# DanEngelbrecht/longtail

Hardware: AMD Instinct MI355X
Metric: ingest GB/s (chunk+hash+compress) (higher is better)
Workload: dtype u8/u32

## Files before the change

longtail_amd/csrc/k_lz4.hip:

```cpp
#include "k_copy.h"
#include "lthip_internal.h"

#include <string>

#include <stdlib.h>

namespace
{

struct Lz4Block
{
    uint64_t src_off;
    uint64_t dst_off;
    uint32_t size;
    uint32_t dst_cap;
    uint32_t seg_base;
    uint32_t nseg;
    uint32_t grp_base;
    uint32_t ngrp;
    uint32_t cgrp_base;
    uint32_t ncgrp;
};

struct Lz4Meta
// ... 115 lines not shown
        uint4 o;
        if constexpr (PAD)
        {
            const uint32_t w = b >> 2, sh = b & 3u;
            uint32_t d[4];
            lds_run<true, 4>(sdata, w, d);
            const uint32_t d4 = lds_dw<true>(sdata, w + 4u);
            o.x = __builtin_amdgcn_alignbyte(d[1], d[0], sh);
            o.y = __builtin_amdgcn_alignbyte(d[2], d[1], sh);
            o.z = __builtin_amdgcn_alignbyte(d[3], d[2], sh);
            o.w = __builtin_amdgcn_alignbyte(d4, d[3], sh);
        }
        else
        {
            o.x = lds_read32(sdata, b);
            o.y = lds_read32(sdata, b + 4u);
            o.z = lds_read32(sdata, b + 8u);
            o.w = lds_read32(sdata, b + 12u);
        }
        *reinterpret_cast<uint4*>(dst + (uint64_t)v * 16u) = o;
    }
    const uint32_t done = nvec << 4;
    if ((uint32_t)lane < n - done)
        dst[done + (uint32_t)lane] = (uint8_t)lds_byte<PAD>(sdata, sbyte + done + (uint32_t)lane);
}

__device__ __forceinline__ void emit_len(uint8_t* out, uint32_t len, int lane)
{
    const uint32_t n = len / 255u + 1u;
    for (uint32_t j = lane; j < n; j += 64)
        out[j] = j + 1 == n ? (uint8_t)(len % 255u) : (uint8_t)255;
}

struct Lz4Seq
{
    uint32_t op;
    uint32_t anchor;
    uint32_t first_lit;
    uint32_t first_hdr;
    uint32_t nseq;
    bool have_first;
};

template <int FMT>
__device__ __forceinline__ void lz4_coop_sequence(const uint8_t* __restrict__ sbytes, uint32_t head, uint8_t* __restrict__ out,
                                                  uint64_t* __restrict__ recs, int lane, uint32_t end_limit, uint32_t pf, uint32_t cf,
                                                  uint32_t mlen, bool extend_fwd, bool extend_back, Lz4Seq& st)
{
    if (extend_fwd || extend_back)
    {
        const uint32_t room = extend_back ? (pf - st.anchor < cf ? pf - st.anchor : cf) : 0u;
        uint32_t nf, nb;
        {
            const uint32_t j = (uint32_t)lane & 31u;
            const bool fwd = lane < 32;
            const uint32_t a1 = fwd ? pf + mlen + j : pf - 1u - j;
            const uint32_t a2 = fwd ? cf + mlen + j : cf - 1u - j;
            const bool inr = fwd ? (extend_fwd && a1 < end_limit) : j < room;
            bool same = false;
            if (inr)
                same = sbytes[a1 + head] == sbytes[a2 + head];
            const uint64_t diff = __builtin_amdgcn_ballot_w64(!same);
            const uint32_t dl = (uint32_t)diff, dh = (uint32_t)(diff >> 32);
            nf = dl ? (uint32_t)__builtin_ctz(dl) : 32u;
            nb = dh ? (uint32_t)__builtin_ctz(dh) : 32u;
        }
        mlen += nf;
        if (nf == 32u)
        {
            const uint32_t* sdata = reinterpret_cast<const uint32_t*>(sbytes);
            for (;;)
            {
                const uint32_t i = pf + mlen + 4u * (uint32_t)lane;
                uint32_t cnt = 0;
                if (i < end_limit)
                {
                    const uint32_t x = lds_read32(sdata, i + head) ^ lds_read32(sdata, cf + mlen + 4u * (uint32_t)lane + head);
                    const uint32_t lim = end_limit - i < 4u ? end_limit - i : 4u;
                    cnt = x ? (uint32_t)__builtin_ctz(x) >> 3 : 4u;
                    cnt = cnt < lim ? cnt : lim;
                }
                const uint64_t diff = __builtin_amdgcn_ballot_w64(cnt < 4u);
                if (diff)
                {
                    const int f = __builtin_ctzll(diff);
                    mlen += 4u * (uint32_t)f + __builtin_amdgcn_readlane(cnt, f);
                    break;
                }
                mlen += 256u;
            }
        }
        if (nb == 32u && room > 32u)
        {
            uint32_t back = 32u;
            for (;;)
            {
                const uint32_t j = back + (uint32_t)lane;
                const bool same = j < room && sbytes[pf - 1u - j + head] == sbytes[cf - 1u - j + head];
                const uint64_t diff = __builtin_amdgcn_ballot_w64(!same);
                if (diff)
                {
                    back += (uint32_t)__builtin_ctzll(diff);
                    break;
                }
                back += 64u;
            }
            nb = back;
        }
        pf -= nb;
        cf -= nb;
        mlen += nb;
    }
    const uint32_t lit = pf - st.anchor;
    const uint32_t mcode = mlen - 4u;
    const uint32_t off = pf - cf;
    if constexpr (FMT == 1)
    {
        for (uint32_t j = lane; j < lit; j += 64)
            out[st.op + j] = sbytes[st.anchor + j + head];
        if (lane == 0)
            recs[st.nseq] = (uint64_t)lit | ((uint64_t)mlen << 16) | ((uint64_t)off << 32);
        st.have_first = true;
        st.nseq += 1u;
        st.op += lit;
        st.anchor = pf + mlen;
        return;
    }
    const uint32_t hdr = 1u + lz4_len_bytes(lit);
    const uint32_t mext = lz4_len_bytes(mcode);
    const uint32_t total = hdr + lit + 2u + mext;
    const uint32_t token = ((lit < 15u ? lit : 15u) << 4) | (mcode < 15u ? mcode : 15u);
    for (uint32_t j = lane; j < total; j += 64)
    {
        uint32_t b;
        if (j >= hdr && j < hdr + lit)
            b = sbytes[st.anchor + (j - hdr) + head];
        else if (j == 0)
            b = token;
        else if (j < hdr)
            b = j + 1 == hdr ? (lit - 15u) % 255u : 255u;
        else if (j == hdr + lit)
            b = off & 255u;
        else if (j == hdr + lit + 1u)
            b = off >> 8;
        else
            b = j + 1 == total ? (mcode - 15u) % 255u : 255u;
        out[st.op + j] = (uint8_t)b;
    }
    if (!st.have_first)
    {
        st.have_first = true;
        st.first_lit = lit;
        st.first_hdr = hdr;
    }
    st.op += total;
    st.anchor = pf + mlen;
}

constexpr int LZ4_G_BATCH = 8;
constexpr int LZ4_G_LANES = 16;
constexpr int LZ4_PROBE_BATCHES = 4;
constexpr uint32_t LZ4_Z_CHAIN = LTHIP_ZSTD_CHAIN;
constexpr uint32_t Z_PIECE = 128u << 10;
constexpr int LZ4_TAB_LZ4 = 1024 + 256;
constexpr int LZ4_TAB_ZSTD = 1024 + 256;
[[maybe_unused]] constexpr int LZ4_TAB_LANES = 2560;
constexpr int LZ4_TAB_SHARED = 1536, LZ4_SH_LOG2 = 13;

#include "lz4/lz4_lane_parse.inc"
#include "lz4/lz4_classify.inc"
#include "lz4/lz4_lanes_kernel.inc"
#include "lz4/lz4_stitch.inc"


}


extern "C" size_t lthip_lz4_bound(size_t size) { return size > 0x7E000000u ? 0 : size + size / 255 + 16; }

static int upload_blocks(lthip_ctx* ctx, uint32_t block_count, const uint64_t* src_offsets, const uint32_t* src_sizes,
                         const uint64_t* dst_offsets, const uint32_t* dst_caps, uint32_t seg_bytes, uint32_t gunits, Lz4Block** d_blocks,
                         uint64_t* out_nseg, uint64_t* out_ngrp = nullptr, uint64_t* out_ncgrp = nullptr)
{
    std::vector<Lz4Block> hb(block_count);
    uint64_t nseg = 0, ngrp = 0, ncgrp = 0;
    for (uint32_t b = 0; b < block_count; ++b)
    {
        if (src_sizes[b] > 0x7E000000u)
            return lthip_fail(ctx, EINVAL, "lz4", "block larger than LZ4_MAX_INPUT_SIZE");
        hb[b].src_off = src_offsets[b];
        hb[b].dst_off = dst_offsets[b];
        hb[b].size = src_sizes[b];
        hb[b].dst_cap = dst_caps[b];
        hb[b].seg_base = (uint32_t)nseg;
        hb[b].nseg = seg_bytes ? (uint32_t)(((uint64_t)src_sizes[b] + seg_bytes - 1) / seg_bytes) : 0;
        hb[b].grp_base = (uint32_t)ngrp;
        hb[b].ngrp = (hb[b].nseg + gunits - 1) / gunits;
        ngrp += hb[b].ngrp;
        hb[b].cgrp_base = (uint32_t)ncgrp;
        hb[b].ncgrp = (hb[b].nseg + LZ4_G_BATCH - 1) / LZ4_G_BATCH;
        ncgrp += hb[b].ncgrp;
        nseg += hb[b].nseg;
    }
    if (nseg > 0x7FFFFFF0ull)
        return lthip_fail(ctx, EINVAL, "lz4", "too many segments in one batch");
    void* p;
    int err = lthip_scratch(ctx, S_LZ4_BLOCKS, sizeof(Lz4Block) * (size_t)block_count, &p);
    if (err)
        return err;
    if ((err = lthip_stage_upload(ctx, p, hb.data(), sizeof(Lz4Block) * (size_t)block_count, ctx->stream)))
        return err;
    *d_blocks = (Lz4Block*)p;
    *out_nseg = nseg;
    if (out_ngrp)
        *out_ngrp = ngrp;
    if (out_ncgrp)
        *out_ncgrp = ncgrp;
    return 0;
}

#ifdef LTHIP_K5_PROF
extern "C" __attribute__((visibility("default"))) int lthip_k5_prof_dump(int reset)
{
    unsigned long long h[32];
    if (hipMemcpyFromSymbol(h, HIP_SYMBOL(g_k5_prof), sizeof(h)) != hipSuccess)
        return -1;
    static const char* names[16] = {"stage+clear+barrier", "prefetch issue", "pre-seed", "loop: probe", "loop: extend fwd/back", "loop: long+record",
                                    "cover scans", "emission", "unit end", "group barrier", "#probe iterations", "#extension rounds", "#hits", "#long matches", "", ""};
    unsigned long long tot = 0;
    for (int i = 0; i < 10; ++i)
        tot += h[i];
    for (int i = 0; i < 14; ++i)
        printf("k5prof %-24s %14llu%s\n", names[i], h[i], i < 10 ? (std::string("  ") + std::to_string(100.0 * (double)h[i] / (double)(tot ? tot : 1)).substr(0, 5) + " %").c_str() : "");
    if (reset)
    {
        memset(h, 0, sizeof(h));
        (void)hipMemcpyToSymbol(HIP_SYMBOL(g_k5_prof), h, sizeof(h));
    }
    return 0;
}
#endif

static bool lz4_lane_parser()
{
#ifdef LTHIP_ABLATIONS
    static const bool v = [] {
        const char* e = getenv("LTHIP_LZ4_PARSER");
        return !(e && strcmp(e, "batch") == 0);
    }();
    return v;
#else
    return true;
#endif
}

template <int FMT, int CLS>
static int launch_segments(lthip_ctx* ctx, uint32_t groups, uint32_t SEG, const void* d_src, const Lz4Block* d_blocks, uint32_t block_count,
                           uint32_t g0, uint8_t* streams, Lz4Meta* meta, uint64_t* zrecs, uint8_t* spec_dst, uint32_t dbg, uint32_t ngroups,
                           uint32_t* worklist)
{
    constexpr int TAB = FMT == 1 ? LZ4_TAB_ZSTD : LZ4_TAB_LZ4;
    const size_t lds = (size_t)lz4_window_lds_bytes(LZ4_G_BATCH * SEG + 64u, false) + 16 + (size_t)LZ4_G_BATCH * TAB * 2;
    if (lds > 64u * 1024u && !ctx->k5_lds_enabled[FMT][CLS])
    {
        LTHIP_CHECK(ctx, hipFuncSetAttribute(reinterpret_cast<const void*>(&k_lz4_segments<LZ4_G_BATCH, TAB, FMT, CLS>),
                                             hipFuncAttributeMaxDynamicSharedMemorySize, 160 * 1024));
        ctx->k5_lds_enabled[FMT][CLS] = true;
    }
    hipLaunchKernelGGL((k_lz4_segments<LZ4_G_BATCH, TAB, FMT, CLS>), dim3(groups), dim3(64 * LZ4_G_BATCH), lds, ctx->stream, (const uint8_t*)d_src,
                       d_blocks, block_count, g0, SEG, streams, meta, zrecs, spec_dst, dbg, nullptr, ngroups, worklist);
    LTHIP_LAUNCH_CHECK(ctx);
    return 0;
}

#ifdef LTHIP_ABLATIONS
template <int TAB, int FMT, int SH = 0, int PV = 0>
static int launch_segments_lane_mode(lthip_ctx* ctx, uint32_t groups, uint32_t SEG, const void* d_src, const Lz4Block* d_blocks, uint32_t block_count,
                                     uint8_t* streams, Lz4Meta* meta, uint64_t* zrecs, uint8_t* spec_dst, uint32_t dbg, uint64_t* lane_recs,
                                     uint32_t ngroups, uint32_t* worklist)
{
    constexpr int G = LZ4_G_LANES;
    const size_t lds = (size_t)lz4_window_lds_bytes(G * SEG + 64u + (PV == 2 ? LZ4_LPAD : 0u), PV == 2) + 16 + (size_t)G * TAB * 2 + (SH ? (size_t)4 << SH : 0);
    static bool granted[64] = {};
    if (ctx->device < 0 || ctx->device >= 64 || !granted[ctx->device])
    {
        LTHIP_CHECK(ctx, hipFuncSetAttribute(reinterpret_cast<const void*>(&k_lz4_segments_modes<G, TAB, FMT, 1, 0, SH, PV>),
                                             hipFuncAttributeMaxDynamicSharedMemorySize, 160 * 1024));
        if (ctx->device >= 0 && ctx->device < 64)
            granted[ctx->device] = true;
    }
    int ncu = 256;
    (void)hipDeviceGetAttribute(&ncu, hipDeviceAttributeMultiprocessorCount, ctx->device);
    const uint32_t grid = groups < (uint32_t)ncu ? groups : (uint32_t)ncu;
    hipLaunchKernelGGL((k_lz4_segments_modes<G, TAB, FMT, 1, 0, SH, PV>), dim3(grid), dim3(64 * G), lds, ctx->stream, (const uint8_t*)d_src, d_blocks,
                       block_count, 0u, SEG, streams, meta, zrecs, spec_dst, dbg, lane_recs, ngroups, worklist);
    LTHIP_LAUNCH_CHECK(ctx);
    return 0;
}
#endif

template <int FMT>
static int launch_match_finder(lthip_ctx* ctx, bool lanes, uint32_t SEG, const void* d_src, const Lz4Block* d_blocks, uint32_t block_count,
                               uint32_t g0, uint32_t g1, uint64_t ngrp, uint64_t ncgrp, uint8_t* streams, Lz4Meta* meta, uint64_t* zrecs,
                               uint8_t* spec_dst, uint32_t dbg, [[maybe_unused]] uint64_t* lane_recs)
{
    if (!lanes)
        return launch_segments<FMT, 0>(ctx, g1 - g0, SEG, d_src, d_blocks, block_count, g0, streams, meta, zrecs, spec_dst, dbg, 0, nullptr);
#ifdef LTHIP_ABLATIONS
    LTHIP_ABLATION_ENV(env_shared, "LTHIP_LZ4_SHARED");
    const bool shared = env_shared.get() != 0;
    LTHIP_ABLATION_ENV(env_pv, "LTHIP_LZ4_PV");
    const bool pv2 = shared && env_pv.get() != 0;
    if (dbg & 16384u)
        return pv2      ? launch_segments_lane_mode<LZ4_TAB_SHARED, FMT, LZ4_SH_LOG2, 2>(ctx, (uint32_t)ngrp, SEG, d_src, d_blocks, block_count, streams, meta, zrecs,
                                                                                        spec_dst, dbg, lane_recs, (uint32_t)ngrp, nullptr)
               : shared ? launch_segments_lane_mode<LZ4_TAB_SHARED, FMT, LZ4_SH_LOG2>(ctx, (uint32_t)ngrp, SEG, d_src, d_blocks, block_count, streams, meta, zrecs,
                                                                                     spec_dst, dbg, lane_recs, (uint32_t)ngrp, nullptr)
                        : launch_segments_lane_mode<LZ4_TAB_LANES, FMT>(ctx, (uint32_t)ngrp, SEG, d_src, d_blocks, block_count, streams, meta, zrecs, spec_dst,
                                                                        dbg, lane_recs, (uint32_t)ngrp, nullptr);
#endif
    void* wl;
    int err = lthip_scratch(ctx, S_LZ4_CLASSIFY, 4 * (11 * (size_t)ngrp + 16), &wl);
    if (err)
        return err;
    LTHIP_CHECK(ctx, hipMemsetAsync(wl, 0, 4 * (2 * (size_t)ngrp + 4), ctx->stream));
    if ((err = launch_segments<FMT, 1>(ctx, (uint32_t)ncgrp, SEG, d_src, d_blocks, block_count, 0, streams, meta, zrecs, spec_dst, dbg, (uint32_t)ngrp,
                                       (uint32_t*)wl)))
        return err;
#ifdef LTHIP_ABLATIONS
    LTHIP_ABLATION_ENV(env_halves, "LTHIP_LZ4_HALVES");
    if (!pv2 || env_halves.get() == 0)
        return pv2      ? launch_segments_lane_mode<LZ4_TAB_SHARED, FMT, LZ4_SH_LOG2, 2>(ctx, (uint32_t)ngrp, SEG, d_src, d_blocks, block_count, streams, meta, zrecs,
                                                                                        spec_dst, dbg, lane_recs, (uint32_t)ngrp, (uint32_t*)wl)
               : shared ? launch_segments_lane_mode<LZ4_TAB_SHARED, FMT, LZ4_SH_LOG2>(ctx, (uint32_t)ngrp, SEG, d_src, d_blocks, block_count, streams, meta, zrecs,
                                                                                     spec_dst, dbg, lane_recs, (uint32_t)ngrp, (uint32_t*)wl)
                        : launch_segments_lane_mode<LZ4_TAB_LANES, FMT>(ctx, (uint32_t)ngrp, SEG, d_src, d_blocks, block_count, streams, meta, zrecs, spec_dst,
                                                                        dbg, lane_recs, (uint32_t)ngrp, (uint32_t*)wl);
#endif
    const uint32_t nthreads = 256, ng = (uint32_t)ngrp;
    uint32_t hist = (FMT == 1 && (dbg & LZ4_DBG_Q_MAX)) ? 3u : (FMT == 1 && (dbg & LZ4_DBG_Q_HIGH)) ? 1u : 0u;
    int ncu = 256;
    (void)hipDeviceGetAttribute(&ncu, hipDeviceAttributeMultiprocessorCount, ctx->device);
    LTHIP_ABLATION_ENV(env_far, "LTHIP_LZ4_FAR");
    const uint32_t farlog = env_far.get() >= 0 ? (uint32_t)env_far.get() : (10u | (12u << 8) | (8u << 16));
#ifdef LTHIP_ABLATIONS
    LTHIP_ABLATION_ENV(env_split, "LTHIP_LZ4_SPLITWG");
    if (env_split.get() > 0 && hist == 0u)
    {
        hist = 2u;
        hipLaunchKernelGGL(k_lz4_pair_halves, dim3((ng + nthreads - 1) / nthreads), dim3(nthreads), 0, ctx->stream, (uint32_t*)wl, ng, 0u, d_blocks, block_count, hist);
        hipLaunchKernelGGL(k_lz4_pair_halves, dim3((2u * ng + nthreads) / nthreads), dim3(nthreads), 0, ctx->stream, (uint32_t*)wl, ng, 1u, d_blocks, block_count, hist);
        LTHIP_LAUNCH_CHECK(ctx);
        const size_t lds8 = (size_t)lz4_window_lds_bytes(8u * SEG + 64u + LZ4_LPAD + 32u, true) + 16 + (size_t)8 * LZ4_TAB_SHARED * 2 + ((size_t)2 << LZ4_SH_LOG2);
        static bool granted8[2] = {false, false};
        if (!granted8[FMT])
        {
            LTHIP_CHECK(ctx, hipFuncSetAttribute(reinterpret_cast<const void*>(&k_lz4_lanes2<FMT, 8>), hipFuncAttributeMaxDynamicSharedMemorySize, 160 * 1024));
            granted8[FMT] = true;
        }
        hipLaunchKernelGGL((k_lz4_lanes2<FMT, 8>), dim3(2u * (uint32_t)ncu), dim3(64 * 8), lds8, ctx->stream, (const uint8_t*)d_src, d_blocks, block_count, SEG,
                           streams, meta, zrecs, spec_dst, dbg, ng, (uint32_t*)wl, farlog);
        LTHIP_LAUNCH_CHECK(ctx);
        return 0;
    }
#endif
    hipLaunchKernelGGL(k_lz4_pair_halves, dim3((ng + nthreads - 1) / nthreads), dim3(nthreads), 0, ctx->stream, (uint32_t*)wl, ng, 0u, d_blocks, block_count, hist);
    hipLaunchKernelGGL(k_lz4_pair_halves, dim3((ng / 2 + nthreads) / nthreads), dim3(nthreads), 0, ctx->stream, (uint32_t*)wl, ng, 1u, d_blocks, block_count, hist);
    LTHIP_LAUNCH_CHECK(ctx);
    const size_t lds = (size_t)lz4_window_lds_bytes(LZ4_G_LANES * SEG + 64u + LZ4_LPAD + 32u, true) + 16 + (size_t)LZ4_G_LANES * LZ4_TAB_SHARED * 2 +
                       ((size_t)4 << LZ4_SH_LOG2);
    if (!ctx->k5h_lds_enabled[FMT])
    {
        LTHIP_CHECK(ctx, hipFuncSetAttribute(reinterpret_cast<const void*>(&k_lz4_lanes2<FMT>), hipFuncAttributeMaxDynamicSharedMemorySize, 160 * 1024));
        ctx->k5h_lds_enabled[FMT] = true;
    }
    hipLaunchKernelGGL((k_lz4_lanes2<FMT>), dim3((uint32_t)ncu), dim3(64 * LZ4_G_LANES), lds, ctx->stream, (const uint8_t*)d_src, d_blocks,
                       block_count, SEG, streams, meta, zrecs, spec_dst, dbg, ng, (uint32_t*)wl, farlog);
    LTHIP_LAUNCH_CHECK(ctx);
    return 0;
}

static int lz4_compress_batch(lthip_ctx* ctx, const void* d_src, uint32_t block_count, const uint64_t* src_offsets,
                              const uint32_t* src_sizes, void* d_dst, const uint64_t* dst_offsets, const uint32_t* dst_caps,
                              uint32_t* d_out_sizes, int segment_log2);

uint64_t lthip_codec_batch_bytes()
{
    static const uint64_t v = [] {
        const char* e = getenv("LTHIP_BATCH_BYTES");
        const uint64_t x = e ? strtoull(e, nullptr, 10) : 0;
        return x ? x : (8ull << 30);
    }();
    return v;
}

uint64_t lthip_origin_budget_mib()
{
    static LthipEnvInt env_org{"LTHIP_ORIGIN_MIB"};
    if (env_org.get() > 0)
        return (uint64_t)env_org.get();
    static const uint64_t v = [] {
        size_t free_b = 0, total_b = 0;
        if (hipMemGetInfo(&free_b, &total_b) != hipSuccess)
            return (uint64_t)4096;
        uint64_t mib = (uint64_t)(free_b >> 20) / 4u;
        mib = mib < 4096u ? 4096u : mib > 16384u ? 16384u : mib;
        return mib;
    }();
    return v;
}

extern "C" int lthip_lz4_compress_blocks(lthip_ctx* ctx, const void* d_src, uint32_t block_count, const uint64_t* src_offsets,
                                         const uint32_t* src_sizes, void* d_dst, const uint64_t* dst_offsets,
                                         const uint32_t* dst_caps, uint32_t* d_out_sizes, int segment_log2)
{
    if (!ctx || !d_out_sizes || (block_count && (!src_offsets || !src_sizes || !dst_offsets || !dst_caps || !d_dst)))
        return EINVAL;
    const uint64_t budget = lthip_codec_batch_bytes();
    for (uint32_t b0 = 0; b0 < block_count;)
    {
        uint64_t bytes = src_sizes[b0];
        uint32_t b1 = b0 + 1;
        while (b1 < block_count && bytes + src_sizes[b1] <= budget)
            bytes += src_sizes[b1++];
        const int err = lz4_compress_batch(ctx, d_src, b1 - b0, src_offsets + b0, src_sizes + b0, d_dst, dst_offsets + b0, dst_caps + b0,
                                           d_out_sizes + b0, segment_log2);
        if (err)
            return err;
        b0 = b1;
    }
    return 0;
}

static int lz4_compress_batch(lthip_ctx* ctx, const void* d_src, uint32_t block_count, const uint64_t* src_offsets,
                              const uint32_t* src_sizes, void* d_dst, const uint64_t* dst_offsets, const uint32_t* dst_caps,
                              uint32_t* d_out_sizes, int segment_log2)
{
    if (segment_log2 == 0)
        segment_log2 = 12;
    if (segment_log2 < 10 || segment_log2 > 13)
        return lthip_fail(ctx, EINVAL, "lz4", "segment_log2 (unit size) must be 0 (default = 12) or 10..13");
    const uint32_t SEG = 1u << segment_log2;
    LTHIP_CHECK(ctx, hipSetDevice(ctx->device));
    Lz4Block* d_blocks = nullptr;
    uint64_t nseg64 = 0, ngrp64 = 0;
    const bool lanes = lz4_lane_parser() && SEG == 4096u;
    const uint32_t GU = lanes ? LZ4_G_LANES : LZ4_G_BATCH;
    uint64_t ncgrp64 = 0;
    int err = upload_blocks(ctx, block_count, src_offsets, src_sizes, dst_offsets, dst_caps, SEG, GU, &d_blocks, &nseg64, &ngrp64, &ncgrp64);
    if (err)
        return err;
    const uint32_t nseg = (uint32_t)nseg64;
    void *meta, *plan, *bout, *streams, *runs, *lrecs = nullptr;
    if (lanes && (err = lthip_scratch(ctx, S_LZ4_LANE_RECS, (size_t)64 * LZ4_LANE_MAXREC * 8 * ((size_t)nseg + 1), &lrecs)))
        return err;
    if ((err = lthip_scratch(ctx, S_TABLES2, 4 * ((size_t)nseg + block_count + 1), &runs)))
        return err;
    if ((err = lthip_scratch(ctx, S_LZ4_META, sizeof(Lz4Meta) * ((size_t)nseg + 1), &meta)))
        return err;
    if ((err = lthip_scratch(ctx, S_LZ4_SEGS, sizeof(Lz4Plan) * ((size_t)nseg + 1), &plan)))
        return err;
    if ((err = lthip_scratch(ctx, S_MISC, sizeof(Lz4BlockOut) * (size_t)block_count, &bout)))
        return err;
    if ((err = lthip_scratch(ctx, S_LZ4_STREAM, (size_t)lz4_stream_stride(SEG) * ((size_t)nseg + 1), &streams)))
        return err;
    LTHIP_ABLATION_ENV(env_dbg, "LTHIP_LZ4_DBG");
    const uint32_t dbg = env_dbg.get() > 0 ? (uint32_t)env_dbg.get() : 0u;
    uint64_t total_bytes = 0;
    for (uint32_t b = 0; b < block_count; ++b)
        total_bytes += src_sizes[b];
    const uint32_t want = (!(dbg & 32u) || lanes) ? 1u : (total_bytes >= (1ull << 30) ? 4u : (total_bytes >= (256ull << 20) ? 2u : 1u));
    std::vector<uint32_t> cut{0};
    {
        uint64_t acc = 0;
        for (uint32_t b = 0; b < block_count; ++b)
        {
            acc += src_sizes[b];
            if (cut.size() < want && acc * want >= total_bytes * cut.size() && b + 1 < block_count)
                cut.push_back(b + 1);
        }
        cut.push_back(block_count);
    }
    std::vector<uint32_t> grp_first(block_count + 1, 0);
    for (uint32_t b = 0; b < block_count; ++b)
        grp_first[b + 1] = grp_first[b] + (uint32_t)(((((uint64_t)src_sizes[b] + SEG - 1) / SEG) + GU - 1) / GU);
    const bool overlap = cut.size() > 2;
    void* worklist;
    if ((err = lthip_scratch(ctx, S_LZ4_WORKLIST, 4 * (2 * (size_t)ngrp64 + 1) * (cut.size() - 1), &worklist)))
        return err;
    int ncu = 256;
    (void)hipDeviceGetAttribute(&ncu, hipDeviceAttributeMultiprocessorCount, ctx->device);
    LTHIP_ABLATION_ENV(env_swg, "LTHIP_LZ4_STITCH_WGS");
    int stitch_wgs = 7;
    if (hipOccupancyMaxActiveBlocksPerMultiprocessor(&stitch_wgs, k_lz4_stitch_copy, K6_THREADS, 0) != hipSuccess || stitch_wgs < 1)
        stitch_wgs = 7;
    const uint32_t copy_grid = (uint32_t)ncu * (env_swg.get() > 0 ? (uint32_t)env_swg.get() : 2u * (uint32_t)stitch_wgs);
    hipStream_t s2 = ctx->stream;
    if (overlap)
    {
        if ((err = lthip_second_stream(ctx, &s2)))
            return err;
    }
    for (size_t i = 0; i + 1 < cut.size(); ++i)
    {
        const uint32_t b0 = cut[i], b1 = cut[i + 1];
        const uint32_t g0 = grp_first[b0], g1 = grp_first[b1];
        if (g1 > g0)
        {
            LaunchTimer t(ctx, LTHIP_K_LZ4_SEG);
            uint8_t* spec = (dbg & 64u) ? (uint8_t*)nullptr : (uint8_t*)d_dst;
            if ((err = launch_match_finder<0>(ctx, lanes, SEG, d_src, d_blocks, block_count, g0, g1, ngrp64, ncgrp64, (uint8_t*)streams, (Lz4Meta*)meta,
                                              nullptr, spec, dbg, (uint64_t*)lrecs)))
                return err;
        }
        if (overlap)
        {
            hipEvent_t e = lthip_sync_event(ctx);
            LTHIP_CHECK(ctx, hipEventRecord(e, ctx->stream));
            LTHIP_CHECK(ctx, hipStreamWaitEvent(s2, e, 0));
        }
        {
            LaunchTimer t(ctx, LTHIP_K_LZ4_STITCH, s2);
            uint32_t* wl = (uint32_t*)worklist + (size_t)i * (2 * (size_t)ngrp64 + 1);
            LTHIP_CHECK(ctx, hipMemsetAsync(wl, 0, 4, s2));
            hipLaunchKernelGGL(k_lz4_stitch_scan, dim3(b1 - b0), dim3(64), 0, s2, d_blocks, b0, b1, SEG, (const Lz4Meta*)meta,
                               (Lz4Plan*)plan, (uint32_t*)runs, (Lz4BlockOut*)bout, d_out_sizes, (uint8_t*)d_dst, (dbg & 64u) ? 0u : 1u, wl, (uint32_t)ngrp64);
            if (g1 > g0)
                hipLaunchKernelGGL(k_lz4_stitch_copy, dim3(g1 - g0 < copy_grid ? g1 - g0 : copy_grid), dim3(K6_THREADS), 0, s2,
                                   (const uint8_t*)d_src, d_blocks, block_count, SEG, (const uint8_t*)streams, (const Lz4Meta*)meta,
                                   (const Lz4Plan*)plan, (const uint32_t*)runs, (const Lz4BlockOut*)bout, (uint8_t*)d_dst,
                                   (const uint32_t*)wl, GU, (uint32_t)ngrp64);
            if (i + 2 == cut.size())
                hipLaunchKernelGGL(k_lz4_empty_blocks, dim3((block_count + 255) / 256), dim3(256), 0, s2, d_blocks, block_count,
                                   (const Lz4BlockOut*)bout, (uint8_t*)d_dst);
            LTHIP_LAUNCH_CHECK(ctx);
        }
    }
    if (overlap)
    {
        hipEvent_t e = lthip_sync_event(ctx);
        LTHIP_CHECK(ctx, hipEventRecord(e, s2));
        LTHIP_CHECK(ctx, hipStreamWaitEvent(ctx->stream, e, 0));
    }
    return 0;
}

int lthip_launch_lz_sequences(lthip_ctx* ctx, const void* d_src, uint32_t block_count, const uint64_t* src_offsets,
                              const uint32_t* src_sizes, void* d_dst, const uint64_t* dst_offsets, const uint32_t* dst_caps,
                              uint8_t** d_lits, uint64_t** d_recs, void** d_meta, uint32_t* unit_base, uint64_t* total_units, int quality)
{
    const uint32_t SEG = 4096u;
    Lz4Block* d_blocks = nullptr;
    uint64_t nseg64 = 0, ngrp64 = 0;
    const bool lanes = lz4_lane_parser();
    uint64_t ncgrp64 = 0;
    int err = upload_blocks(ctx, block_count, src_offsets, src_sizes, dst_offsets, dst_caps, SEG, lanes ? LZ4_G_LANES : LZ4_G_BATCH, &d_blocks,
                            &nseg64, &ngrp64, &ncgrp64);
    if (err)
        return err;
    uint64_t nseg = 0;
    for (uint32_t b = 0; b < block_count; ++b)
    {
        unit_base[b] = (uint32_t)nseg;
        nseg += ((uint64_t)src_sizes[b] + SEG - 1) / SEG;
    }
    *total_units = nseg;
    void *lits, *recs, *meta;
    if ((err = lthip_scratch(ctx, S_Z_LITS, (size_t)SEG * (nseg + 1), &lits)))
        return err;
    if ((err = lthip_scratch(ctx, S_Z_RECS, (size_t)SEG * 2 * (nseg + 1), &recs)))
        return err;
    if ((err = lthip_scratch(ctx, S_LZ4_META, sizeof(Lz4Meta) * ((size_t)nseg + 1), &meta)))
        return err;
    void* lrecs = nullptr;
    if (lanes && (err = lthip_scratch(ctx, S_LZ4_LANE_RECS, (size_t)64 * LZ4_LANE_MAXREC * 8 * ((size_t)nseg + 1), &lrecs)))
        return err;
    if (nseg)
    {
        LaunchTimer t(ctx, LTHIP_K_LZ4_SEG);
        LTHIP_ABLATION_ENV(env_dbg, "LTHIP_LZ4_DBG");
        uint32_t dbg = env_dbg.get() > 0 ? (uint32_t)env_dbg.get() : 0u;
        if (quality >= 1)
            dbg |= LZ4_DBG_Q_HIGH;
        if (quality >= 2)
            dbg |= LZ4_DBG_Q_MAX;
        if ((err = launch_match_finder<1>(ctx, lanes, SEG, d_src, d_blocks, block_count, 0u, (uint32_t)ngrp64, ngrp64, ncgrp64, (uint8_t*)lits,
                                          (Lz4Meta*)meta, (uint64_t*)recs, (uint8_t*)d_dst, dbg, (uint64_t*)lrecs)))
            return err;
    }
    *d_lits = (uint8_t*)lits;
    *d_recs = (uint64_t*)recs;
    *d_meta = meta;
    return 0;
}
```

longtail_amd/csrc/lz4/lz4_classify.inc:

```
template <int G, int TAB, int FMT, int CLS = 0>
__global__ __launch_bounds__(64 * G, 6) void k_lz4_segments(const uint8_t* __restrict__ src, const Lz4Block* __restrict__ blocks,
                                                             uint32_t nblocks, uint32_t grp0, uint32_t sub_bytes,
                                                             uint8_t* __restrict__ streams, Lz4Meta* __restrict__ meta,
                                                             uint64_t* __restrict__ zrecs, uint8_t* __restrict__ spec_dst, uint32_t dbg,
                                                             uint64_t* __restrict__ lane_recs, uint32_t ngroups, uint32_t* __restrict__ worklist)
{
    extern __shared__ __attribute__((aligned(16))) uint32_t smem[];
    constexpr bool PAD = false;
    const uint32_t data_bytes = lz4_window_lds_bytes(G * sub_bytes + 64u, PAD);
    uint32_t* sdata = smem;
    const uint8_t* sbytes = reinterpret_cast<const uint8_t*>(sdata);
    uint32_t* flag = reinterpret_cast<uint32_t*>(reinterpret_cast<uint8_t*>(smem) + data_bytes);
    const int tid = threadIdx.x;
    const int lane = tid & 63;
    const int wave = __builtin_amdgcn_readfirstlane(tid >> 6);
    uint16_t* tab = reinterpret_cast<uint16_t*>(reinterpret_cast<uint8_t*>(smem) + data_bytes + 16u) + (size_t)wave * TAB;
    K5P_DECL
    {
    const uint32_t grp = grp0 + blockIdx.x;
    uint32_t lo = 0, hi = nblocks;
    while (hi - lo > 1)
    {
        const uint32_t mid = lo + ((hi - lo) >> 1);
        if ((CLS ? blocks[mid].cgrp_base : blocks[mid].grp_base) <= grp)
            lo = mid;
        else
            hi = mid;
    }
    const Lz4Block blk = blocks[lo];
    const uint32_t gi = grp - (CLS ? blk.cgrp_base : blk.grp_base);
    const uint32_t group_start = gi * G * sub_bytes;
    const uint32_t glen = blk.size - group_start < G * sub_bytes ? blk.size - group_start : G * sub_bytes;
    const uint8_t* g = src + blk.src_off + group_start;

    const uint32_t head_src = (uint32_t)((uintptr_t)g & 15u);
    const uint32_t head = head_src;
    {
        const uint4* gv = reinterpret_cast<const uint4*>(g - head_src);
        const uint32_t nvec = (head_src + glen + 15u) >> 4;
        uint4* sv = reinterpret_cast<uint4*>(sdata);
        for (uint32_t v0 = 0; v0 < nvec; v0 += 64 * G * 4)
        {
            uint4 q[4];
#pragma unroll
            for (int u = 0; u < 4; ++u)
            {
                const uint32_t v = v0 + u * 64 * G + tid;
                q[u] = v < nvec ? gv[v] : make_uint4(0, 0, 0, 0);
            }
#pragma unroll
            for (int u = 0; u < 4; ++u)
            {
                const uint32_t v = v0 + u * 64 * G + tid;
                if (v < nvec)
                    sv[v] = q[u];
            }
        }
        uint4* tv = reinterpret_cast<uint4*>(tab);
        const uint32_t e1 = 0xFFFFFFFFu;
        const uint4 e = make_uint4(e1, e1, e1, e1);
#pragma unroll
        for (uint32_t v = 0; v < (TAB * 2 / 16 + 63) / 64; ++v)
            if (v * 64 + lane < TAB * 2 / 16)
                tv[v * 64 + lane] = e;
        if (tid == 0)
            *flag = 0u;
    }
    __syncthreads();
    K5P(0);

    K5P(1);
    const uint32_t my_start = (uint32_t)wave * sub_bytes;
    const bool have_unit = my_start < glen;
    const bool emit_unit = have_unit;
    const uint32_t my_len = have_unit ? (glen - my_start < sub_bytes ? glen - my_start : sub_bytes) : 0u;
    const uint32_t unit = blk.seg_base + gi * G + (uint32_t)wave;
    const int64_t blk_left = (int64_t)blk.size - (int64_t)group_start - (int64_t)my_start;
    int64_t sl = (int64_t)my_len - 4;
    if (sl > blk_left - 12)
        sl = blk_left - 12;
    const int32_t start_limit = have_unit ? (int32_t)((int64_t)my_start + sl) : -1;
    const int64_t el = (int64_t)my_len < blk_left - 5 ? (int64_t)my_len : (blk_left - 5 > 0 ? blk_left - 5 : 0);
    const uint32_t end_limit = my_start + (uint32_t)el;

    uint8_t* out = streams + (uint64_t)unit * (FMT == 1 ? sub_bytes : lz4_stream_stride(sub_bytes));
    uint64_t* recs = FMT == 1 ? zrecs + (uint64_t)unit * (sub_bytes >> 2) : nullptr;
    Lz4Seq st;
    st.op = 0;
    st.nseq = 0;
    st.anchor = my_start;
    st.first_lit = st.first_hdr = 0;
    st.have_first = false;
    uint32_t pos = my_start, nfail = 0;
    bool met = false;
    uint32_t batches = 0;
    uint32_t pb0 = 0, pb1 = 0, pb2 = 0, pb3 = 0, ps0 = 1, ps1 = 1, ps2 = 1, ps3 = 1;
    static_assert(LZ4_PROBE_BATCHES == 4, "probe bookkeeping is unrolled by hand");

    for (;;)
    {
        const bool more = have_unit && (int32_t)pos <= start_limit;
        if (!met && (batches == LZ4_PROBE_BATCHES || !more))
        {
            if (st.have_first && lane == 0)
                *flag = 1u;
            __syncthreads();
            if constexpr (CLS != 0)
            {
                if (*flag != 0u)
                {
                    if (tid == 0)
                    {
                        const uint32_t g16 = blk.grp_base + gi / (uint32_t)(LZ4_G_LANES / LZ4_G_BATCH);
#ifdef LTHIP_ABLATIONS
                        if (atomicOr(&worklist[1u + ngroups + g16], 1u << (gi & 1u)) == 0u)
                            worklist[1u + atomicAdd(&worklist[0], 1u)] = g16;
#else
                        (void)__hip_atomic_fetch_or(&worklist[1u + ngroups + g16], 1u << (gi & 1u), __ATOMIC_RELAXED, __HIP_MEMORY_SCOPE_AGENT);
#endif
                    }
                    return;
                }
            }
            if (*flag != 0u && wave != 0 && have_unit && !(dbg & 1u))
            {
                for (uint32_t q0 = 0; q0 < my_start; q0 += 1024)
                {
                    uint32_t hv[4];
#pragma unroll
                    for (int u = 0; u < 4; ++u)
                        hv[u] = __umulhi(lds_read32(sdata, q0 + 4u * (u * 64 + (uint32_t)lane) + head) * 2654435761u, (uint32_t)TAB);
#pragma unroll
                    for (int u = 0; u < 4; ++u)
                        tab[hv[u]] = (uint16_t)(q0 + 4u * (u * 64 + (uint32_t)lane));
                }
#define LT_REPLAY(r, PB, PS)                                                                            \
    if ((r) < batches)                                                                                  \
    {                                                                                                   \
        const uint32_t rp = (PB) + (uint32_t)lane * (PS);                                               \
        if ((int32_t)rp <= start_limit)                                                                 \
            tab[__umulhi(lds_read32(sdata, rp + head) * 2654435761u, (uint32_t)TAB)] = (uint16_t)rp;         \
    }
                LT_REPLAY(0u, pb0, ps0)
                LT_REPLAY(1u, pb1, ps1)
                LT_REPLAY(2u, pb2, ps2)
                LT_REPLAY(3u, pb3, ps3)
#undef LT_REPLAY
            }
            else if (*flag == 0u && more && !(dbg & 16u))
                nfail += 24u;
            met = true;
        }
        if (!more)
            break;
        if (batches == 0) { pb0 = pos; ps0 = 1u + nfail; }
        else if (batches == 1) { pb1 = pos; ps1 = 1u + nfail; }
        else if (batches == 2) { pb2 = pos; ps2 = 1u + nfail; }
        else if (batches == 3) { pb3 = pos; ps3 = 1u + nfail; }
        ++batches;

        uint32_t stride = 1u + nfail;
        uint32_t p = pos + (uint32_t)lane * stride;
        bool valid = (int32_t)p <= start_limit;
        uint32_t v = 0, cand = LZ4_EMPTY, h = 0;
        bool ok = false;
        if (met && nfail != 0u && !(dbg & 8u))
        {
            const uint32_t pos2 = pos + 64u * stride;
            const uint32_t p2 = pos2 + (uint32_t)lane * (stride + 1u);
            const bool valid2 = (int32_t)p2 <= start_limit;
            uint32_t v2 = 0, cand2 = LZ4_EMPTY, h2 = 0;
            if (valid)
            {
                v = lds_read32(sdata, p + head);
                h = __umulhi(v * 2654435761u, (uint32_t)TAB);
                cand = tab[h];
            }
            if (valid2)
            {
                v2 = lds_read32(sdata, p2 + head);
                h2 = __umulhi(v2 * 2654435761u, (uint32_t)TAB);
                cand2 = tab[h2];
            }
            if (valid)
                tab[h] = (uint16_t)p;
            bool ok2 = false;
            if (valid && cand != LZ4_EMPTY && cand < p)
                ok = lds_read32(sdata, cand + head) == v;
            if (valid2 && cand2 != LZ4_EMPTY && cand2 < p2)
                ok2 = lds_read32(sdata, cand2 + head) == v2;
            if (__builtin_amdgcn_ballot_w64(ok) == 0ull)
            {
                if (valid2)
                    tab[h2] = (uint16_t)p2;
                if (__builtin_amdgcn_ballot_w64(ok2) == 0ull)
                {
                    pos = pos2 + 64u * (stride + 1u);
                    nfail += 2u;
                    continue;
                }
                pos = pos2;
                ++nfail;
                stride += 1u;
                p = p2;
                cand = cand2;
                ok = ok2;
            }
        }
        else
        {
            if (valid)
            {
                v = lds_read32(sdata, p + head);
                h = __umulhi(v * 2654435761u, (uint32_t)TAB);
                cand = tab[h];
            }
            if (valid)
                tab[h] = (uint16_t)p;
            if (valid && cand != LZ4_EMPTY && cand < p)
                ok = lds_read32(sdata, cand + head) == v;
        }
        if (nfail == 0 && !(dbg & 2u))
        {
            uint32_t best = 0;
            bool found = false;
            uint32_t ovs[4];
#pragma unroll
            for (int t = 0; t < 4; ++t)
                ovs[t] = __shfl_up(v, 8 >> t, 64);
#pragma unroll
            for (int t = 0; t < 4; ++t)
            {
                const int d = 8 >> t;
                if (valid && lane >= d && ovs[t] == v)
                {
                    best = p - (uint32_t)d * stride;
                    found = true;
                }
            }
            if (found && (!ok || best > cand))
            {
                cand = best;
                ok = true;
            }
        }
        uint64_t hits = __builtin_amdgcn_ballot_w64(ok);
        if (hits == 0ull)
        {
            pos += 64u * stride;
            ++nfail;
            continue;
        }
        if constexpr (CLS != 0)
        {
            if (!met)
            {
                st.have_first = true;
                if (lane == 0)
                    *flag = 1u;
                pos = (uint32_t)(start_limit + 1);
                continue;
            }
        }
        if (dbg & 4u)
        {
            do
            {
                const int f = __builtin_ctzll(hits);
                hits &= hits - 1ull;
                const uint32_t pf = pos + (uint32_t)f * stride;
                if (pf < st.anchor)
                    continue;
                lz4_coop_sequence<FMT>(sbytes, head, out, recs, lane, end_limit, pf, __builtin_amdgcn_readlane(cand, f), 4u, true, true, st);
            } while (hits);
            const uint32_t np = pos + 64u * stride;
            pos = np > st.anchor ? np : st.anchor;
            nfail = 0;
            continue;
        }
        if (stride != 1u)
        {
            const int f = __builtin_ctzll(hits);
            lz4_coop_sequence<FMT>(sbytes, head, out, recs, lane, end_limit, pos + (uint32_t)f * stride, __builtin_amdgcn_readlane(cand, f), 4u,
                              true, true, st);
            pos = st.anchor;
            nfail = 0;
            continue;
        }
        uint32_t mlen = ok ? 4u : 0u;
        bool act = ok;
        const uint32_t maxlen = ok ? end_limit - p : 0u;
#pragma unroll 1
        for (int t = 0; t < 2; ++t)
        {
            if (__builtin_amdgcn_ballot_w64(act) == 0ull)
                break;
            if (act)
            {
                const uint32_t a0 = p + mlen + head, b0 = cand + mlen + head;
                const uint32_t x0 = lds_read32(sdata, a0) ^ lds_read32(sdata, b0);
                const uint32_t x1 = lds_read32(sdata, a0 + 4u) ^ lds_read32(sdata, b0 + 4u);
                const uint32_t x2 = lds_read32(sdata, a0 + 8u) ^ lds_read32(sdata, b0 + 8u);
                const uint32_t x3 = lds_read32(sdata, a0 + 12u) ^ lds_read32(sdata, b0 + 12u);
                uint32_t add = 16u;
                if (x0)
                    add = (uint32_t)__builtin_ctz(x0) >> 3;
                else if (x1)
                    add = 4u + ((uint32_t)__builtin_ctz(x1) >> 3);
                else if (x2)
                    add = 8u + ((uint32_t)__builtin_ctz(x2) >> 3);
                else if (x3)
                    add = 12u + ((uint32_t)__builtin_ctz(x3) >> 3);
                mlen += add;
                if (add != 16u)
                    act = false;
                if (mlen >= maxlen)
                {
                    mlen = maxlen;
                    act = false;
                }
            }
        }
        const uint64_t longs = __builtin_amdgcn_ballot_w64(act);
        uint32_t nbk = 0;
        if (ok && cand >= 8u)
        {
            const uint32_t x = lds_read32(sdata, p - 4u + head) ^ lds_read32(sdata, cand - 4u + head);
            const uint32_t y = lds_read32(sdata, p - 8u + head) ^ lds_read32(sdata, cand - 8u + head);
            nbk = x ? (uint32_t)__builtin_clz(x) >> 3 : (y ? 4u + ((uint32_t)__builtin_clz(y) >> 3) : 8u);
        }
        uint64_t rem = hits, vecsel = 0ull;
        uint32_t sel_v = 0;
        while (rem)
        {
            if (st.anchor > pos)
            {
                const uint32_t sh = st.anchor - pos;
                rem = sh >= 64u ? 0ull : rem & (~0ull << sh);
                if (!rem)
                    break;
            }
            const int f = __builtin_ctzll(rem);
            rem &= rem - 1ull;
            const uint32_t pf = pos + (uint32_t)f;
            const bool isl = (longs >> f) & 1ull;
            const uint32_t room = pf - st.anchor;
            if (isl || room > 20u)
            {
                lz4_coop_sequence<FMT>(sbytes, head, out, recs, lane, end_limit, pf, __builtin_amdgcn_readlane(cand, f),
                                  __builtin_amdgcn_readlane(mlen, f), isl, true, st);
                continue;
            }
            uint32_t nb = __builtin_amdgcn_readlane(nbk, f);
            nb = nb < room ? nb : room;
            const uint32_t lit = room - nb;
            const uint32_t len = __builtin_amdgcn_readlane(mlen, f) + nb;
            if (lit > 12u)
            {
                lz4_coop_sequence<FMT>(sbytes, head, out, recs, lane, end_limit, pf - nb, __builtin_amdgcn_readlane(cand, f) - nb, len, false,
                                  false, st);
                continue;
            }
            sel_v = lane == f ? (FMT == 1 ? st.nseq << 20 : 0u) | (st.op << 8) | (nb << 4) | lit : sel_v;
            vecsel |= 1ull << f;
            if (!st.have_first)
            {
                st.have_first = true;
                st.first_lit = lit;
                st.first_hdr = 1u;
            }
            if constexpr (FMT == 1)
            {
                st.op += lit;
                st.nseq += 1u;
            }
            else
                st.op += lit + 3u + (len - 4u >= 15u ? 1u : 0u);
            st.anchor = pf + len - nb;
        }
        if ((vecsel >> lane) & 1ull)
        {
            const uint32_t lit = sel_v & 15u;
            const uint32_t nb = (sel_v >> 4) & 15u;
            const uint32_t lit_start_v = p - nb - lit;
            const uint32_t off = p - cand;
            if constexpr (FMT == 1)
            {
                uint8_t* o = out + ((sel_v >> 8) & 0xFFFu);
                for (uint32_t j = 0; j < lit; ++j)
                    o[j] = sbytes[lit_start_v + j + head];
                recs[sel_v >> 20] = (uint64_t)lit | ((uint64_t)(mlen + nb) << 16) | ((uint64_t)off << 32);
            }
            else
            {
                const uint32_t mcode = mlen + nb - 4u;
                uint8_t* o = out + (sel_v >> 8);
                o[0] = (uint8_t)((lit << 4) | (mcode < 15u ? mcode : 15u));
                for (uint32_t j = 0; j < lit; ++j)
                    o[1u + j] = sbytes[lit_start_v + j + head];
                o[1u + lit] = (uint8_t)off;
                o[2u + lit] = (uint8_t)(off >> 8);
                if (mcode >= 15u)
                    o[3u + lit] = (uint8_t)(mcode - 15u);
            }
        }
        const uint32_t np = pos + 64u;
        pos = np > st.anchor ? np : st.anchor;
        nfail = 0;
    }
    if constexpr (FMT == 1)
    {
        const uint32_t tail = emit_unit ? my_start + my_len - st.anchor : 0u;
        if (st.nseq != 0u)
        {
            for (uint32_t j = lane; j < tail; j += 64)
                out[st.op + j] = (uint8_t)lds_byte<PAD>(sdata, st.anchor + j + head);
        }
        else if (emit_unit && spec_dst)
        {
            const uint32_t pos = group_start + my_start;
            const uint64_t o = 13u + (uint64_t)(pos / Z_PIECE) * (Z_PIECE + 3u) + 3u + pos % Z_PIECE;
            if (o + my_len <= (uint64_t)blk.dst_cap)
                wave_copy_lds_to_global<PAD>(spec_dst + blk.dst_off + o, sdata, my_start + head, my_len, lane);
        }
        uint32_t uniform = 0;
        if (emit_unit)
        {
            const uint32_t b0 = lds_byte<PAD>(sdata, my_start + head);
            const uint32_t rep = b0 * 0x01010101u;
            uint32_t diff = 0;
            if (64u * (uint32_t)lane + 4u <= my_len)
                diff = lds_read32x<PAD>(sdata, my_start + 64u * (uint32_t)lane + head) ^ rep;
            if (__builtin_amdgcn_ballot_w64(diff != 0u) == 0ull)
#pragma unroll 4
            for (uint32_t j = 0; j < 16u; ++j)
            {
                const uint32_t o = 64u * (uint32_t)lane + 4u * j;
                if (o + 4u <= my_len)
                    diff |= lds_read32x<PAD>(sdata, my_start + o + head) ^ rep;
                else if (o < my_len)
                    for (uint32_t k = o; k < my_len; ++k)
                        diff |= lds_byte<PAD>(sdata, my_start + k + head) ^ b0;
            }
            uniform = __builtin_amdgcn_ballot_w64(diff != 0u) == 0ull ? (0x100u | b0) : 0u;
        }
        if (emit_unit && lane == 0)
            reinterpret_cast<uint4*>(meta)[unit] = make_uint4(st.nseq, st.op + tail, tail, uniform);
    }
    else
    {
    if (FMT == 0 && spec_dst && emit_unit && !st.have_first)
    {
        const uint64_t o = (uint64_t)(1u + lz4_len_bytes(blk.size)) + group_start + my_start;
        if (o + my_len <= (uint64_t)blk.dst_cap)
            wave_copy_lds_to_global<PAD>(spec_dst + blk.dst_off + o, sdata, my_start + head, my_len, lane);
    }
    if (emit_unit && lane == 0)
    {
        Lz4Meta m;
        m.seq_bytes = st.op;
        m.tail_lits = my_start + my_len - st.anchor;
        m.first_lit_len = st.first_lit;
        m.first_hdr_bytes = st.first_hdr;
        meta[unit] = m;
    }
    }
    K5P(8);
    K5P(9);
    }
}

#ifdef LTHIP_ABLATIONS
#include "../ablations/k_lz4_segments_modes.inc"
#endif
```

longtail_amd/csrc/lz4/lz4_stitch.inc:

```
__device__ __forceinline__ void wg_emit_header(uint8_t* dst, uint32_t lits, uint32_t match_nibble, int tid, int nthreads)
{
    if (tid == 0)
        dst[0] = (uint8_t)(((lits < 15u ? lits : 15u) << 4) | match_nibble);
    if (lits >= 15u)
    {
        const uint32_t len = lits - 15u;
        const uint32_t n = len / 255u + 1u;
        for (uint32_t j = tid; j < n; j += nthreads)
            dst[1 + j] = j + 1 == n ? (uint8_t)(len % 255u) : (uint8_t)255;
    }
}

__global__ __launch_bounds__(64) void k_lz4_stitch_scan(const Lz4Block* __restrict__ blocks, uint32_t b0, uint32_t nblocks, uint32_t SEG,
                                                        const Lz4Meta* __restrict__ meta, Lz4Plan* __restrict__ plan,
                                                        uint32_t* __restrict__ runs, Lz4BlockOut* __restrict__ bout,
                                                        uint32_t* __restrict__ out_sizes, uint8_t* __restrict__ dst, uint32_t spec,
                                                        uint32_t* __restrict__ worklist ,
                                                        uint32_t wl_cap)
{
    const uint32_t b = blockIdx.x + b0;
    if (b >= nblocks)
        return;
    const int lane = threadIdx.x;
    const Lz4Block blk = blocks[b];
    const uint32_t run_base = blk.seg_base + b;
    uint64_t out_pos = 0;
    uint32_t carry = 0;
    uint32_t run = 0;
    Lz4Meta m;
    m.seq_bytes = m.tail_lits = m.first_lit_len = m.first_hdr_bytes = 0;
    if ((uint32_t)lane < blk.nseg)
        m = meta[blk.seg_base + (uint32_t)lane];
    for (uint32_t i0 = 0; i0 < blk.nseg; i0 += 64)
    {
        const uint32_t i = i0 + (uint32_t)lane;
        const Lz4Meta cur = m;
        if (i + 64u < blk.nseg)
            m = meta[blk.seg_base + i + 64u];
        const bool valid = i < blk.nseg;
        const bool has = valid && cur.seq_bytes != 0u;
        const uint32_t seg_len = valid ? (blk.size - i * SEG < SEG ? blk.size - i * SEG : SEG) : 0u;
        uint32_t sv = has ? cur.tail_lits : seg_len;
        uint32_t sf = has ? 1u : 0u;
#pragma unroll
        for (int d = 1; d < 64; d <<= 1)
        {
            const uint32_t pv = __shfl_up(sv, d, 64);
            const uint32_t pf = __shfl_up(sf, d, 64);
            if (lane >= d)
            {
                if (!sf)
                    sv += pv;
                sf |= pf;
            }
        }
        if (!sf)
            sv += carry;
        uint32_t cin = __shfl_up(sv, 1, 64);
        if (lane == 0)
            cin = carry;
        const uint32_t L = cin + cur.first_lit_len;
        const uint32_t hdr = 1u + lz4_len_bytes(L);
        const uint64_t adv = has ? (uint64_t)hdr + L + (cur.seq_bytes - cur.first_hdr_bytes - cur.first_lit_len) : 0ull;
        uint64_t pos = adv;
#pragma unroll
        for (int d = 1; d < 64; d <<= 1)
        {
            const uint64_t pv = __shfl_up(pos, d, 64);
            if (lane >= d)
                pos += pv;
        }
        const uint64_t my_pos = out_pos + pos - adv;
        const uint64_t hm = __builtin_amdgcn_ballot_w64(has);
        const uint32_t before = (uint32_t)__builtin_popcountll(hm & ((1ull << lane) - 1ull));
        Lz4Plan pl;
        pl.hdr_pos = 0xFFFFFFFFu;
        pl.hdr_lits = pl.first_lit_dst = pl.body_dst = 0;
        pl.tail_rel = cin;
        pl.run = run_base + run + before;
        if (has)
        {
            const uint64_t lit_dst = my_pos + hdr;
            runs[run_base + run + before] = (uint32_t)lit_dst;
            pl.hdr_pos = (uint32_t)my_pos;
            pl.hdr_lits = L;
            pl.first_lit_dst = (uint32_t)(lit_dst + cin);
            pl.body_dst = pl.first_lit_dst + cur.first_lit_len;
            pl.tail_rel = 0;
            pl.run = run_base + run + before + 1u;
        }
        if (valid)
            plan[blk.seg_base + i] = pl;
        out_pos += __shfl(pos, 63, 64);
        carry = __shfl(sv, 63, 64);
        run += (uint32_t)__builtin_popcountll(hm);
    }
    const uint32_t hdr = 1u + lz4_len_bytes(carry);
    const uint64_t lit_dst = out_pos + hdr;
    const uint64_t total = lit_dst + carry;
    if (total <= (uint64_t)blk.dst_cap)
    {
        if (run == 0u && spec)
        {
            if (blk.nseg)
                wg_emit_header(dst + blk.dst_off + out_pos, carry, 0u, lane, 64);
        }
        else
        {
            uint32_t base = 0;
            if (lane == 0)
                base = atomicAdd(worklist, blk.ngrp);
            base = __builtin_amdgcn_readfirstlane(base);
            for (uint32_t k = lane; k < blk.ngrp; k += 64)
            {
                worklist[1u + base + k] = blk.grp_base + k;
                worklist[1u + wl_cap + base + k] = b;
            }
        }
    }
    if (lane == 0)
    {
        runs[run_base + run] = (uint32_t)lit_dst;
        Lz4BlockOut bo;
        bo.final_hdr_pos = (uint32_t)out_pos;
        bo.final_lits = carry;
        bo.total = total <= (uint64_t)blk.dst_cap ? (uint32_t)total : 0u;
        bo.pad = run == 0u ? 1u : 0u;
        bout[b] = bo;
        out_sizes[b] = bo.total;
    }
}

__device__ __forceinline__ void wg_copy(uint8_t* __restrict__ dst, const uint8_t* __restrict__ src, uint32_t n, int lane)
{
    if (n)
        lthip_wg_copy<64>(dst, src, n, lane);
}

constexpr int K6_THREADS = 256;

#ifdef LTHIP_K6_WAVES
__attribute__((amdgpu_waves_per_eu(LTHIP_K6_WAVES, LTHIP_K6_WAVES)))
#endif
__global__ __launch_bounds__(K6_THREADS) void k_lz4_stitch_copy(const uint8_t* __restrict__ src,
                                                                 const Lz4Block* __restrict__ blocks, uint32_t nblocks,
                                                                 uint32_t SEG, const uint8_t* __restrict__ streams,
                                                                 const Lz4Meta* __restrict__ meta,
                                                                 const Lz4Plan* __restrict__ plan,
                                                                 const uint32_t* __restrict__ runs,
                                                                 const Lz4BlockOut* __restrict__ bout,
                                                                 uint8_t* __restrict__ dst, const uint32_t* __restrict__ worklist,
                                                                 uint32_t gunits , uint32_t wl_cap)
{
    const int tid = threadIdx.x;
    const uint32_t nwork = worklist[0];
    (void)nblocks;
  for (uint32_t wi = blockIdx.x; wi < nwork; wi += gridDim.x)
  {
    const uint32_t grp = worklist[1u + wi];
    const uint32_t lo = worklist[1u + wl_cap + wi];
    const Lz4Block blk = blocks[lo];
    const Lz4BlockOut bo = bout[lo];
    uint8_t* d = dst + blk.dst_off;
    const uint32_t i0 = (grp - blk.grp_base) * gunits;
    const uint32_t i1 = i0 + gunits < blk.nseg ? i0 + gunits : blk.nseg;
    const int lane = tid & 63;
    for (uint32_t i = i0 + (uint32_t)(tid >> 6); i < i1; i += K6_THREADS / 64)
    {
        const uint32_t seg = blk.seg_base + i;
        const uint32_t seg_start = i * SEG;
        const uint32_t len = blk.size - seg_start < SEG ? blk.size - seg_start : SEG;
        const Lz4Meta m = meta[seg];
        const Lz4Plan pl = plan[seg];
        const uint8_t* s = src + blk.src_off + seg_start;
        const uint8_t* stream = streams + (uint64_t)seg * lz4_stream_stride(SEG);
        uint32_t tail = len;
        if (m.seq_bytes)
        {
            wg_emit_header(d + pl.hdr_pos, pl.hdr_lits, stream[0] & 15u, lane, 64);
            wg_copy(d + pl.first_lit_dst, s, m.first_lit_len, lane);
            const uint32_t skip = m.first_hdr_bytes + m.first_lit_len;
            wg_copy(d + pl.body_dst, stream + skip, m.seq_bytes - skip, lane);
            tail = m.tail_lits;
        }
        wg_copy(d + runs[pl.run] + pl.tail_rel, s + (len - tail), tail, lane);
        if (i + 1 == blk.nseg)
            wg_emit_header(d + bo.final_hdr_pos, bo.final_lits, 0u, lane, 64);
    }
  }
}

__global__ void k_lz4_empty_blocks(const Lz4Block* __restrict__ blocks, uint32_t nblocks,
                                   const Lz4BlockOut* __restrict__ bout, uint8_t* __restrict__ dst)
{
    const uint32_t b = blockIdx.x * blockDim.x + threadIdx.x;
    if (b >= nblocks)
        return;
    if (blocks[b].nseg == 0 && bout[b].total == 1)
        dst[blocks[b].dst_off] = 0;
}
```

Before: 921.8.

## Fast-path stitch scan for blocks with no matches using classify flags

The classify kernel now sets a flag bit in each group's worklist word when a segment produces sequences. The stitch scan reads these words, and if a whole block has no matches it emits a single literal-run header directly and skips the per-segment walk. A vectorized long-header writer fills the 255-byte runs with 16-byte stores. This adds atomics in classify and depends on the worklist word layout, which is changed so only the low bits gate the worklist push.

```diff
diff --git a/longtail_amd/csrc/k_lz4.hip b/longtail_amd/csrc/k_lz4.hip
--- a/longtail_amd/csrc/k_lz4.hip
+++ b/longtail_amd/csrc/k_lz4.hip
@@ -441,8 +441,10 @@
 template <int FMT>
 static int launch_match_finder(lthip_ctx* ctx, bool lanes, uint32_t SEG, const void* d_src, const Lz4Block* d_blocks, uint32_t block_count,
                                uint32_t g0, uint32_t g1, uint64_t ngrp, uint64_t ncgrp, uint8_t* streams, Lz4Meta* meta, uint64_t* zrecs,
-                               uint8_t* spec_dst, uint32_t dbg, [[maybe_unused]] uint64_t* lane_recs)
-{
+                               uint8_t* spec_dst, uint32_t dbg, [[maybe_unused]] uint64_t* lane_recs, const uint32_t** grp_words = nullptr)
+{
+    if (grp_words)
+        *grp_words = nullptr;
     if (!lanes)
         return launch_segments<FMT, 0>(ctx, g1 - g0, SEG, d_src, d_blocks, block_count, g0, streams, meta, zrecs, spec_dst, dbg, 0, nullptr);
 #ifdef LTHIP_ABLATIONS
@@ -466,6 +468,8 @@
     if ((err = launch_segments<FMT, 1>(ctx, (uint32_t)ncgrp, SEG, d_src, d_blocks, block_count, 0, streams, meta, zrecs, spec_dst, dbg, (uint32_t)ngrp,
                                        (uint32_t*)wl)))
         return err;
+    if (grp_words)
+        *grp_words = (const uint32_t*)wl + 1 + ngrp;
 #ifdef LTHIP_ABLATIONS
     LTHIP_ABLATION_ENV(env_halves, "LTHIP_LZ4_HALVES");
     if (!pv2 || env_halves.get() == 0)
@@ -644,14 +648,18 @@
     {
         const uint32_t b0 = cut[i], b1 = cut[i + 1];
         const uint32_t g0 = grp_first[b0], g1 = grp_first[b1];
+        const uint32_t* grp_words = nullptr;
         if (g1 > g0)
         {
             LaunchTimer t(ctx, LTHIP_K_LZ4_SEG);
             uint8_t* spec = (dbg & 64u) ? (uint8_t*)nullptr : (uint8_t*)d_dst;
             if ((err = launch_match_finder<0>(ctx, lanes, SEG, d_src, d_blocks, block_count, g0, g1, ngrp64, ncgrp64, (uint8_t*)streams, (Lz4Meta*)meta,
-                                              nullptr, spec, dbg, (uint64_t*)lrecs)))
+                                              nullptr, spec, dbg, (uint64_t*)lrecs, &grp_words)))
                 return err;
         }
+        LTHIP_ABLATION_ENV(env_walk, "LTHIP_LZ4_PLAIN_WALK");
+        if ((dbg & 64u) || env_walk.get() > 0)
+            grp_words = nullptr;
         if (overlap)
         {
             hipEvent_t e = lthip_sync_event(ctx);
@@ -663,7 +671,8 @@
             uint32_t* wl = (uint32_t*)worklist + (size_t)i * (2 * (size_t)ngrp64 + 1);
             LTHIP_CHECK(ctx, hipMemsetAsync(wl, 0, 4, s2));
             hipLaunchKernelGGL(k_lz4_stitch_scan, dim3(b1 - b0), dim3(64), 0, s2, d_blocks, b0, b1, SEG, (const Lz4Meta*)meta,
-                               (Lz4Plan*)plan, (uint32_t*)runs, (Lz4BlockOut*)bout, d_out_sizes, (uint8_t*)d_dst, (dbg & 64u) ? 0u : 1u, wl, (uint32_t)ngrp64);
+                               (Lz4Plan*)plan, (uint32_t*)runs, (Lz4BlockOut*)bout, d_out_sizes, (uint8_t*)d_dst, (dbg & 64u) ? 0u : 1u, wl, (uint32_t)ngrp64,
+                               grp_words);
             if (g1 > g0)
                 hipLaunchKernelGGL(k_lz4_stitch_copy, dim3(g1 - g0 < copy_grid ? g1 - g0 : copy_grid), dim3(K6_THREADS), 0, s2,
                                    (const uint8_t*)d_src, d_blocks, block_count, SEG, (const uint8_t*)streams, (const Lz4Meta*)meta,
diff --git a/longtail_amd/csrc/lz4/lz4_classify.inc b/longtail_amd/csrc/lz4/lz4_classify.inc
--- a/longtail_amd/csrc/lz4/lz4_classify.inc
+++ b/longtail_amd/csrc/lz4/lz4_classify.inc
@@ -113,7 +113,7 @@
                     {
                         const uint32_t g16 = blk.grp_base + gi / (uint32_t)(LZ4_G_LANES / LZ4_G_BATCH);
 #ifdef LTHIP_ABLATIONS
-                        if (atomicOr(&worklist[1u + ngroups + g16], 1u << (gi & 1u)) == 0u)
+                        if ((atomicOr(&worklist[1u + ngroups + g16], 1u << (gi & 1u)) & 3u) == 0u)
                             worklist[1u + atomicAdd(&worklist[0], 1u)] = g16;
 #else
                         (void)__hip_atomic_fetch_or(&worklist[1u + ngroups + g16], 1u << (gi & 1u), __ATOMIC_RELAXED, __HIP_MEMORY_SCOPE_AGENT);
@@ -463,6 +463,9 @@
         m.first_lit_len = st.first_lit;
         m.first_hdr_bytes = st.first_hdr;
         meta[unit] = m;
+        if (CLS != 0 && st.op != 0u)
+            (void)__hip_atomic_fetch_or(&worklist[1u + ngroups + blk.grp_base + gi / (uint32_t)(LZ4_G_LANES / LZ4_G_BATCH)], 4u, __ATOMIC_RELAXED,
+                                        __HIP_MEMORY_SCOPE_AGENT);
     }
     }
     K5P(8);
diff --git a/longtail_amd/csrc/lz4/lz4_stitch.inc b/longtail_amd/csrc/lz4/lz4_stitch.inc
--- a/longtail_amd/csrc/lz4/lz4_stitch.inc
+++ b/longtail_amd/csrc/lz4/lz4_stitch.inc
@@ -9,6 +9,32 @@
         for (uint32_t j = tid; j < n; j += nthreads)
             dst[1 + j] = j + 1 == n ? (uint8_t)(len % 255u) : (uint8_t)255;
     }
+}
+__device__ __forceinline__ void wave_emit_long_header(uint8_t* dst, uint32_t lits, int lane)
+{
+    if (lits < 15u + 255u * 64u)
+    {
+        wg_emit_header(dst, lits, 0u, lane, 64);
+        return;
+    }
+    const uint32_t len = lits - 15u;
+    const uint32_t n255 = len / 255u;
+    uint8_t* p = dst + 1;
+    const uint32_t headb = (uint32_t)((16u - ((uintptr_t)p & 15u)) & 15u);
+    if (lane == 0)
+        dst[0] = (uint8_t)(15u << 4);
+    if ((uint32_t)lane < headb)
+        p[lane] = (uint8_t)255;
+    const uint32_t nvec = (n255 - headb) >> 4;
+    uint4* pv = reinterpret_cast<uint4*>(p + headb);
+    const uint4 ff = make_uint4(0xFFFFFFFFu, 0xFFFFFFFFu, 0xFFFFFFFFu, 0xFFFFFFFFu);
+    for (uint32_t v = (uint32_t)lane; v < nvec; v += 64u)
+        pv[v] = ff;
+    const uint32_t done = headb + (nvec << 4);
+    if ((uint32_t)lane < n255 - done)
+        p[done + (uint32_t)lane] = (uint8_t)255;
+    if (lane == 0)
+        p[n255] = (uint8_t)(len % 255u);
 }
 
 __global__ __launch_bounds__(64) void k_lz4_stitch_scan(const Lz4Block* __restrict__ blocks, uint32_t b0, uint32_t nblocks, uint32_t SEG,
@@ -16,7 +42,8 @@
                                                         uint32_t* __restrict__ runs, Lz4BlockOut* __restrict__ bout,
                                                         uint32_t* __restrict__ out_sizes, uint8_t* __restrict__ dst, uint32_t spec,
                                                         uint32_t* __restrict__ worklist ,
-                                                        uint32_t wl_cap)
+                                                        uint32_t wl_cap,
+                                                        const uint32_t* __restrict__ grp_words )
 {
     const uint32_t b = blockIdx.x + b0;
     if (b >= nblocks)
@@ -24,6 +51,34 @@
     const int lane = threadIdx.x;
     const Lz4Block blk = blocks[b];
     const uint32_t run_base = blk.seg_base + b;
+    bool plain = grp_words != nullptr;
+    if (plain)
+    {
+        uint32_t any = 0;
+        for (uint32_t k = (uint32_t)lane; k < blk.ngrp; k += 64u)
+            any |= grp_words[blk.grp_base + k];
+        plain = __builtin_amdgcn_ballot_w64(any != 0u) == 0ull;
+    }
+    if (plain)
+    {
+        const uint32_t hdr = 1u + lz4_len_bytes(blk.size);
+        const uint64_t total = (uint64_t)hdr + blk.size;
+        const bool fits = total <= (uint64_t)blk.dst_cap;
+        if (fits && blk.nseg)
+            wave_emit_long_header(dst + blk.dst_off, blk.size, lane);
+        if (lane == 0)
+        {
+            runs[run_base] = hdr;
+            Lz4BlockOut bo;
+            bo.final_hdr_pos = 0u;
+            bo.final_lits = blk.size;
+            bo.total = fits ? (uint32_t)total : 0u;
+            bo.pad = 1u;
+            bout[b] = bo;
+            out_sizes[b] = bo.total;
+        }
+        return;
+    }
     uint64_t out_pos = 0;
     uint32_t carry = 0;
     uint32_t run = 0;
@@ -103,7 +158,7 @@
         if (run == 0u && spec)
         {
             if (blk.nseg)
-                wg_emit_header(dst + blk.dst_off + out_pos, carry, 0u, lane, 64);
+                wave_emit_long_header(dst + blk.dst_off + out_pos, carry, lane);
         }
         else
         {
```

New measurement: 923.6, median of 4. No clear change (+0.2%).
